# mozilla/mozjpeg

Hardware: AMD Instinct MI355X
Metric: Mpixels/s encode (4K RGB q75 trellis) at 1/2/4/8 GPUs; bit-exact vs cjpeg (higher is better)
Workload: dtype u8/int16 (+f32 trellis costs); 1 GPU; 3840x2160 synthetic RGB, q75 4:2:0 baseline, trellis+deringing+optimal Huffman (cjpeg -quality 75 -baseline); config_key=metric, frames_per_encode_call=96, distinct_frames=96, batches_in_flight=2, input=resident in HBM, output=complete JPEG files in HBM, parallelism=images sharded, 1 process per GPU, no collective

## Files before the change

include/mozjpeg_hip.h:

```cpp
#ifndef MOZJPEG_HIP_H
#define MOZJPEG_HIP_H

#include <stddef.h>
#include <stdint.h>

#ifdef __cplusplus
extern "C" {
#endif

#define MJH_MAX_COMPS 4
#define MJH_MAX_SCANS 64

#define MJH_OK            0
#define MJH_EINVAL       -1
#define MJH_EUNSUPPORTED -2
#define MJH_EHIP         -3
#define MJH_ENOMEM       -4
#define MJH_ETOOSMALL    -5

#define MJH_PROFILE_MAX_COMPRESSION 0x5D083AAD
#define MJH_PROFILE_FASTEST         0x2AEA5CB4

typedef struct {
  int comps_in_scan;
// ... 166 lines not shown
  int dct_method;
  int bottom_up;
  int raw_planes;
  int no_dither;
} mjh_decode_opts;
void mjh_decode_opts_defaults(mjh_decode_opts *o);
int mjh_decode_host(mjh_encoder *e, const void *const jpegs[], const size_t sizes[], int n, const mjh_decode_opts *opts);
int mjh_decode_wait(mjh_encoder *e);
int mjh_get_pixels(mjh_encoder *e, int i, void *dst, size_t row_pitch);
int mjh_get_pixels_device(mjh_encoder *e, void **d_base, size_t *row_pitch, size_t *image_stride);
int mjh_get_plane(mjh_encoder *e, int i, int comp, void *dst, size_t row_pitch, int width, int height);
int mjh_get_planes_device(mjh_encoder *e, int comp, void **d_base, size_t *row_pitch, size_t *image_stride, int *width, int *height);
int mjh_decode_stats(mjh_encoder *e, int *width, int *height, int *pixel_size, float ms[2]);

int mjh_enc_onepass_stats(mjh_encoder *e, int *enabled, unsigned long long *long_blocks, unsigned long long *big_groups);

int mjh_get_jpeg_size(mjh_encoder *e, int i, size_t *size);
int mjh_get_jpeg(mjh_encoder *e, int i, void *dst, size_t cap, size_t *size);
int mjh_get_output_device(mjh_encoder *e, void **d_base, size_t *stride, void **d_sizes);

int mjh_get_scan_table(mjh_encoder *e, int image, int scan, int tblno, uint8_t bits[17], uint8_t vals[256]);

enum {
  MJH_TAP_PLANE = 1,
  MJH_TAP_COEF_UQ = 2,
  MJH_TAP_COEF_Q = 3,
  MJH_TAP_COEF_Q0 = 4,
  MJH_TAP_HUFF_BITS = 5,
  MJH_TAP_HUFF_VALS = 6,
  MJH_TAP_PROG_SCAN_US = 7,
// ... 24 lines not shown
```

mozjpeg_amd/__init__.py:

```python
import ctypes as C
import os

import numpy as np

_HERE = os.path.dirname(os.path.abspath(__file__))
LIB_PATH = os.environ.get("MOZJPEG_AMD_LIB") or os.path.join(_HERE, "libmozjpeg_hip.so")

MAX_COMPS, MAX_SCANS = 4, 64
PROFILE_MAX_COMPRESSION = 0x5D083AAD
PROFILE_FASTEST = 0x2AEA5CB4
COLOR_YCC, COLOR_NONE, COLOR_YCC_IN = 0, 1, 2
CS_GRAYSCALE, CS_RGB, CS_YCBCR = 1, 2, 3
CS_RGB565 = 16
OK, EINVAL, EUNSUPPORTED, EHIP, ENOMEM, ETOOSMALL = 0, -1, -2, -3, -4, -5
TAP_PLANE, TAP_COEF_UQ, TAP_COEF_Q, TAP_COEF_Q0, TAP_HUFF_BITS, TAP_HUFF_VALS, TAP_PROG_SCAN_US, TAP_LL_COUNTS = 1, 2, 3, 4, 5, 6, 7, 8


class MjhError(RuntimeError):
    def __init__(self, code, msg):
        super().__init__("mozjpeg_hip error %d: %s" % (code, msg))
        self.code = code


class Scan(C.Structure):
# ... 127 lines not shown
        L.mjh_transcode_host.argtypes = [C.c_void_p, C.POINTER(C.c_char_p), C.POINTER(C.c_size_t), C.c_int]
        L.mjh_transcode_status.argtypes = [C.c_void_p, C.c_int, C.POINTER(C.c_char_p)]
        L.mjh_transcode_stats.argtypes = [C.c_void_p, C.POINTER(C.c_int), C.POINTER(C.c_int), C.POINTER(C.c_int), C.POINTER(C.c_float)]
        if hasattr(L, "mjh_decode_host"):
            L.mjh_decode_opts_defaults.argtypes = [C.POINTER(DecodeOpts)]
            L.mjh_decode_opts_defaults.restype = None
            L.mjh_decode_host.argtypes = [C.c_void_p, C.POINTER(C.c_char_p), C.POINTER(C.c_size_t), C.c_int, C.POINTER(DecodeOpts)]
            L.mjh_get_pixels.argtypes = [C.c_void_p, C.c_int, C.c_void_p, C.c_size_t]
            L.mjh_get_pixels_device.argtypes = [C.c_void_p, C.POINTER(C.c_void_p), C.POINTER(C.c_size_t), C.POINTER(C.c_size_t)]
            L.mjh_decode_stats.argtypes = [C.c_void_p, C.POINTER(C.c_int), C.POINTER(C.c_int), C.POINTER(C.c_int), C.POINTER(C.c_float)]
            L.mjh_decode_wait.argtypes = [C.c_void_p]
            L.mjh_get_plane.argtypes = [C.c_void_p, C.c_int, C.c_int, C.c_void_p, C.c_size_t, C.c_int, C.c_int]
            L.mjh_get_planes_device.argtypes = [C.c_void_p, C.c_int, C.POINTER(C.c_void_p), C.POINTER(C.c_size_t), C.POINTER(C.c_size_t),
                                                C.POINTER(C.c_int), C.POINTER(C.c_int)]
            L.mjh_transcode_batch_size.argtypes = [C.c_void_p]
        if hasattr(L, "mjh_enc_onepass_stats"):
            L.mjh_enc_onepass_stats.argtypes = [C.c_void_p, C.POINTER(C.c_int), C.POINTER(C.c_ulonglong), C.POINTER(C.c_ulonglong)]
        _lib = L
    return _lib


def _chk(rc):
    if rc != 0:
        raise MjhError(rc, lib().mjh_last_error().decode())


def make_params(width, height, *, quality=75, baseline=False, revert=False, optimize=False,
                notrellis=False, notrellis_dc=False, noovershoot=False, sample=(2, 2), gray=False,
                grayin=False, quant_table=-1, lambda1=None, lambda2=None, restart=None,
                progressive=False, fastcrush=False, precision=8, trellis_loops=1, smooth=0, rgb=False,
# ... 550 lines not shown
    def transcode_status(self, i):
        t = C.c_char_p()
        rc = lib().mjh_transcode_status(self._h, i, C.byref(t))
        return rc, (t.value or b"").decode()

    def transcode_stats(self):
        a, b, c, ms = C.c_int(), C.c_int(), C.c_int(), (C.c_float * 4)()
        _chk(lib().mjh_transcode_stats(self._h, C.byref(a), C.byref(b), C.byref(c), ms))
        return dict(subseq=a.value, rounds=b.value, host_syncs=c.value, ms=dict(zip(("sync", "prefix", "store", "dc"), [float(x) for x in ms])))

    def enc_onepass_stats(self):
        on, a, b = C.c_int(), C.c_ulonglong(), C.c_ulonglong()
        _chk(lib().mjh_enc_onepass_stats(self._h, C.byref(on), C.byref(a), C.byref(b)))
        return dict(enabled=bool(on.value), long_blocks=a.value, big_groups=b.value)

    def transcode_host(self, files, errors="raise", **transform):
        n = len(files)
        if transform:
            self.set_transform(transform_spec(**transform))
        try:
            self.submit_transcode(files)
            return [self.get_jpeg(i) for i in range(n)]
        except MjhError:
            if errors != "return":
                raise
            res = self._file_errors(n)
            if res is None:
                raise
            return res

# ... 127 lines not shown
```

mozjpeg_amd/csrc/mjh_encoder.cpp:

```cpp
#include <hip/hip_runtime.h>

#include <math.h>
#include <stdarg.h>
#include <stdio.h>
#include <stdlib.h>
#include <string.h>

#include <atomic>
#include <condition_variable>
#include <functional>
#include <mutex>
#include <string>
#include <thread>
#include <memory>
#include <chrono>
#include <vector>

#include "../../include/mozjpeg_hip.h"
#include "mjh_internal.h"
#include "mjh_launch.h"
#include "mjh_lossless.h"
#include "mjh_decode.h"
#include "mjh_idct.h"
#include "mjh_guard.h"
// ... 243 lines not shown
  uint8_t *d_planes = nullptr;
  int16_t *d_uq = nullptr, *d_q = nullptr, *d_q0 = nullptr;
  MjhQuant *d_quant = nullptr, *d_quant_init = nullptr;
  MjhHuffTable *d_tabs = nullptr, *d_tabs_init = nullptr;
  float *d_lambda = nullptr;
  uint8_t *d_back = nullptr;
  void *d_eob_cost = nullptr; int *d_eob_has = nullptr; long long *d_qsums = nullptr;
  unsigned long long *d_nzmask = nullptr; bool use_compact = false, compact_last = false;
  size_t small_batch = 400000;
  uint8_t *d_nq8 = nullptr;
  int copy_prio = 0;
  int fastdiv_all = 0;
  int dc_mode = 0;
  int dc_late = 1;
  int dc_stats_side = 1;
  int dc_window_ok = 0;
  int trellis_chunks = 0;
  hipEvent_t ev_chunk[4] = { nullptr, nullptr, nullptr, nullptr };
  int trellis_v3 = 4;
  int dqt_off[4] = { -1, -1, -1, -1 };
  int dqt_tabs[4] = { 0, 0, 0, 0 }, dqt_ntab = 0;
  bool tbl_le1 = true;
  int nbands = 1, freq_split = 8;
  unsigned *d_seg_x = nullptr, *d_seg_E = nullptr, *d_seg_sums = nullptr, *d_seg_totals = nullptr, *d_mpos = nullptr;
  int nseg = 1;
  int comp_restart[4] = { 0, 0, 0, 0 };
  int16_t *d_dense = nullptr; unsigned dense_cap = 0;
  unsigned *d_worklist = nullptr, *d_worklist2 = nullptr;
  int trellis_variant = 0;
  bool trellis_adapt = true;
// ... 542 lines not shown
  if (hipStreamSynchronize(a) != hipSuccess || hipStreamSynchronize(b) != hipSuccess) return -1;
  int votes = 0;
  for (int rep = 0; rep < 3; rep++) {
    const auto t0 = std::chrono::steady_clock::now();
    mjh_launch_spin(15000ull, a);
    mjh_launch_spin(15000ull, b);
    if (hipStreamSynchronize(a) != hipSuccess || hipStreamSynchronize(b) != hipSuccess) return -1;
    const double us = std::chrono::duration<double, std::micro>(std::chrono::steady_clock::now() - t0).count();
    votes += us < 240.0;
  }
  return votes >= 2;
}

static thread_local bool g_create_twin = false;
static thread_local int g_twin_onepass = 1;
static thread_local hipStream_t g_twin_avoid[2] = { nullptr, nullptr };

static hipError_t make_streams(mjh_encoder *e)
{
#define STREAMCHK(x) do { const hipError_t r_ = (x); if (r_ != hipSuccess) return r_; } while (0)
  if (e->high_priority_streams) {
    std::vector<hipStream_t> made;
    for (int tries = 0; tries < 12 && !e->side_stream; tries++) {
      hipStream_t c = nullptr;
      STREAMCHK(hipStreamCreateWithFlags(&c, hipStreamNonBlocking));
      made.push_back(c);
      bool free_queue = true;
      for (hipStream_t other : { g_twin_avoid[0], g_twin_avoid[1], e->stream })
        if (other && mjh_streams_overlap(c, other) == 0) { free_queue = false; break; }
      if (!free_queue) continue;
// ... 129 lines not shown
    HIPCHK_E(mjh_dmalloc((void **)&e->d_dense, (size_t)e->dense_cap * 128));
  }
  {
    double m = 0.0;
    for (int k = 1; k < 64; k++) m += p->quantval[p->quant_tbl_no[0]][k];
    m /= 63.0;
    e->trellis_variant = m >= 38.0 ? 0 : m >= 22.0 ? 2 : m >= 13.0 ? 3 : 4;
  }
  if (const char *v = getenv("MJH_TRELLIS_VARIANT")) { e->trellis_variant = atoi(v); e->trellis_adapt = false; }
  HIPCHK_E(hipHostMalloc((void **)&e->h_defer, 64, hipHostMallocDefault));
  if (const char *v = getenv("MJH_TRELLIS_V3")) e->trellis_v3 = atoi(v);
  if (const char *v = getenv("MJH_SMALL_BATCH")) e->small_batch = (size_t)atoll(v);
  if (const char *v = getenv("MJH_TRELLIS_CHUNKS")) { e->trellis_chunks = atoi(v); if (e->trellis_chunks < 0 || e->trellis_chunks > 4) e->trellis_chunks = 0; }
  for (int i = 0; i < 4; i++) HIPCHK_E(hipEventCreateWithFlags(&e->ev_chunk[i], hipEventDisableTiming));
  if (const char *v = getenv("MJH_DC_LATE")) { e->dc_late = atoi(v); if (e->dc_late < 0 || e->dc_late > 2) e->dc_late = 1; }
  e->dc_window_ok = 1;
  for (int i = 0; i < C.ncomp; i++) if (p->quantval[p->quant_tbl_no[i]][0] < 5) e->dc_window_ok = 0;
  if (const char *v = getenv("MJH_DC_SPEC")) e->dc_spec = atoi(v);
  if (const char *v = getenv("MJH_DECODE_SUBSEQ")) { e->dec_subseq = atoi(v); if (e->dec_subseq < 0 || (e->dec_subseq > 0 && e->dec_subseq < 16)) e->dec_subseq = 16; }
  HIPCHK_E(mjh_dmalloc((void **)&e->d_len16, B * (size_t)C.total_mcu_blocks * 2));
  HIPCHK_E(mjh_dmalloc((void **)&e->d_off32, B * (size_t)C.total_mcu_blocks * 4));
  e->chunks = (C.total_mcu_blocks + 2047) / 2048;
  if (g_create_twin) e->enc_onepass = g_twin_onepass;
  else if (const char *v = getenv("MJH_ENC_ONEPASS")) e->enc_onepass = atoi(v) != 0;
  if (e->enc_onepass) {
    e->pack_words = mjh_encode_pack_words(C);
    HIPCHK_E(mjh_dmalloc((void **)&e->d_pack, B * e->pack_words * 4));
    HIPCHK_E(mjh_dmalloc((void **)&e->d_enc_slow, 2 * sizeof(unsigned)));
    HIPCHK_E(hipMemset(e->d_enc_slow, 0, 2 * sizeof(unsigned)));
  }
// ... 436 lines not shown
}

static int run_lossless(mjh_encoder *e, const void *d_pixels, size_t row_pitch, size_t image_stride, int n, hipStream_t s,
                        hipEvent_t input_read, hipEvent_t before_output);

static int run_pipeline(mjh_encoder *e, const void *d_pixels, size_t row_pitch, size_t image_stride, int n, hipStream_t s,
                        const MjhPlaneSrc *plane_src = nullptr, const MjhCoefSrc *coef_src = nullptr,
                        hipEvent_t input_read = nullptr, hipEvent_t before_output = nullptr)
{
  if (e->lossless) return run_lossless(e, d_pixels, row_pitch, image_stride, n, s, input_read, before_output);
  const MjhConst &C = e->C;
  const mjh_params &p = e->p;
  const int spi = e->spi;
  e->sizes_valid = false;
  e->last_n = n;
  e->res_buf = -1;
  e->coef_input = coef_src != nullptr;
  e->last_stream = s;
  if (!e->owner) e->last = nullptr;
  mjh_encoder *const peer = e->owner ? e->owner : e->twin;
  const int if_mode = peer ? (e->owner ? e->owner : e)->inflight_mode : 0;
  const bool ordered = if_mode >= 1;
  if (if_mode == 1 && peer->ev_tier1_set) HIPCHK(hipStreamWaitEvent(s, peer->ev_tier1, 0));
  e->ev_tier1_set = false;
  const bool peer_done_set = peer && peer->ev_done_set;
  if (if_mode == 2) e->ev_done_set = false;
  Prof pr{ e, s };
  if (e->profiling && e->prof_calls < 256) {
    pr.enabled = true;
    pr.first_call = e->prof_calls == 0;
// ... 142 lines not shown
      mjh_launch_prog_stats_par(C, e->d_prog_scans, e->d_lists + plt->par_off, plt->npar, e->d_prog_ctl, e->d_q, e->d_tabs, spi,
                                e->pe, plt->any_refine, nullptr, n, s, plt->nacf);
      pr.mark("gen_tables(trellis)");
      mjh_launch_gen_tables_list(e->d_tabs, spi, e->d_lists + plt->slot_off, plt->nslot, n, s);
      sl_dc = sl_dc_prog;
    }
    if (e->debug_taps && first_pass) {
      if (!e->d_q0) HIPCHK(mjh_dmalloc((void **)&e->d_q0, (size_t)e->max_batch * C.coefs_per_image * 2));
      HIPCHK(hipMemcpyAsync(e->d_q0, e->d_q, (size_t)n * C.coefs_per_image * 2, hipMemcpyDeviceToDevice, s));
    }
    e->side_timed = false;
    bool dc_late = false;
    const int dc_mode = e->dc_mode;
    if (p.trellis_quant_dc && dc_mode == 1) {
      pr.mark("trellis_dc(serial)");
      mjh_launch_trellis_dc(dc_chain_view(e, CV), e->d_quant, e->d_uq, e->d_q, e->d_tabs, spi, sl_dc, e->d_lambda, e->d_back, n, s, e->dc_window_ok);
    } else if (p.trellis_quant_dc) {
      HIPCHK(hipEventRecord(e->ev_fork, s));
      HIPCHK(hipStreamWaitEvent(e->side_stream, e->ev_fork, 0));
      if (pr.enabled && e->profiling == 1) {
        while (e->side_events.size() < 2 * (size_t)(e->prof_calls + 1)) { hipEvent_t ev; HIPCHK(hipEventCreate(&ev)); e->side_events.push_back(ev); }
        HIPCHK(hipEventRecord(e->side_events[2 * e->prof_calls], e->side_stream));
      }
      const size_t spec_bytes = 2 * (size_t)C.total_real_blocks * 9 * 16;
      const bool spec = e->dc_spec && n <= 2 && qstride == 0 && spec_bytes <= ((size_t)256 << 20) && mjh_trellis_dc_speculative_ok(CV, e->dc_window_ok);
      if (spec && !e->d_back9) {
        int rows = 0;
        for (int c = 0; c < C.ncomp; c++) rows += C.c[c].hib;
        HIPCHK(mjh_dmalloc((void **)&e->d_back9, spec_bytes));
        HIPCHK(mjh_dmalloc((void **)&e->d_jfin, 2 * (size_t)rows * 9 * sizeof(int)));
        HIPCHK(mjh_dmalloc((void **)&e->d_qspec, 2 * (size_t)C.total_real_blocks * 9 * sizeof(int16_t)));
      }
      const bool final_dc_here = !e->progressive && p.optimize_coding && last_loop && nbands == 1 && qstride == 0 && !ext_eob && e->dc_stats_side && e->seq_scans.empty();
      const bool sorted_tier = nzm && e->d_nq8 && e->trellis_v3 > 0 && e->trellis_variant <= 4;
      dc_late = e->dc_late > 0 && sorted_tier && !spec && final_dc_here && nloops == 1 && CV.ncomp == 3 && !e->debug_taps && (size_t)n * C.total_real_blocks >= e->small_batch;
      if (spec) mjh_launch_trellis_dc_speculative(CV, e->d_quant, e->d_uq, e->d_q, e->d_tabs, spi, sl_dc, e->d_lambda, e->d_back9, e->d_jfin, e->d_qspec, n, e->side_stream);
      else
      mjh_launch_trellis_dc(dc_chain_view(e, CV), e->d_quant, e->d_uq, e->d_q, e->d_tabs, spi, sl_dc, e->d_lambda, e->d_back, n, e->side_stream, e->dc_window_ok,
                            0, dc_late ? e->dc_late * CV.mcu_rows : -1);
      if (pr.enabled && e->profiling == 1) { HIPCHK(hipEventRecord(e->side_events[2 * e->prof_calls + 1], e->side_stream)); e->side_timed = true; }
      if (final_dc_here && !dc_late) {
        mjh_launch_stats_dc(C, e->d_q, e->d_tabs, spi, fin_dc, 1, zero4, n, e->side_stream);
        final_dc_counted = true;
      }
      if (!dc_late) HIPCHK(hipEventRecord(e->ev_join, e->side_stream));
    }
    const bool extended = nbands > 1 || ext_eob || qstride != 0;
    if (!extended) { const int rc = adapt_first_tier(); if (rc != MJH_OK) return rc; }
    const bool v3 = nzm && e->d_nq8 && e->trellis_v3 > 0 && e->trellis_variant <= 4 && !extended;
    const bool excl = ordered && v3 && !e->progressive;
    if (excl && peer_done_set) HIPCHK(hipStreamWaitEvent(s, peer->ev_done, 0));
    const int trellis_ranges = !v3 || e->debug_taps || (size_t)n * C.total_real_blocks < e->small_batch ? 1
                               : e->trellis_chunks > 0 ? e->trellis_chunks
                               : !e->progressive && (size_t)n * C.total_real_blocks >= (size_t)6000000 ? 2 : 1;
    const int count_mask = v3 && (size_t)n * C.total_real_blocks >= (size_t)2000000 ? 7 : 0;
    pr.mark("trellis_ac");
    mjh_launch_trellis_ac(CV, e->d_quant, e->d_uq, e->d_q, e->d_tabs, spi, sl_ac, e->d_lambda, e->d_worklist, e->d_worklist2, e->d_dense, e->dense_cap,
                          e->trellis_variant,
                          Ss, Se, ext_eob ? e->d_eob_cost : nullptr, ext_eob ? e->d_eob_has : nullptr, nzm, qstride, n, s,
                          e->d_nq8, v3 ? ((size_t)n * C.total_real_blocks < e->small_batch ? 1 : e->trellis_v3) : 0,
                          e->fastdiv_all, dc_late ? e->ev_side0 : nullptr, excl ? e->ev_tier1 : nullptr,
                          trellis_ranges, e->side_stream, e->ev_chunk, count_mask);
    if (excl) e->ev_tier1_set = true;
    if (dc_late) {
      if (!v3) return fail(MJH_EINVAL, "internal: the late DC chains need the tile-sorted trellis' event");
      HIPCHK(hipStreamWaitEvent(e->side_stream, e->ev_side0, 0));
      mjh_launch_trellis_dc(CV, e->d_quant, e->d_uq, e->d_q, e->d_tabs, spi, sl_dc, e->d_lambda, e->d_back, n, e->side_stream, e->dc_window_ok, e->dc_late * CV.mcu_rows, -1);
      mjh_launch_stats_dc(C, e->d_q, e->d_tabs, spi, fin_dc, 1, zero4, n, e->side_stream);
      final_dc_counted = true;
      HIPCHK(hipEventRecord(e->ev_join, e->side_stream));
      join_late = true;
    }
    if (e->trellis_adapt && !extended && first_pass && !e->defer_pending) {
      if (!e->ev_defer) HIPCHK(hipEventCreateWithFlags(&e->ev_defer, hipEventDisableTiming));
      e->defer_frames = n;
      e->defer_scale = count_mask + 1;
      HIPCHK(hipMemcpyAsync(&e->h_defer[0], e->d_worklist, 4 * sizeof(unsigned), hipMemcpyDeviceToHost, s));
      HIPCHK(hipEventRecord(e->ev_defer, s));
      e->defer_pending = true;
    }
    if (ext_eob) {
      pr.mark("trellis_eob_runs");
// ... 165 lines not shown

static mjh_encoder *cur(mjh_encoder *e) { return e && e->last ? e->last : e; }

extern "C" int mjh_set_inflight(mjh_encoder *e, int batches)
{
  if (!e || batches < 1 || batches > 2) return fail(MJH_EINVAL, "batches in flight: 1 or 2");
  e->inflight = batches;
  return MJH_OK;
}

static int make_twin(mjh_encoder *e)
{
  mjh_encoder *t = nullptr;
  g_create_twin = true;
  g_twin_onepass = e->enc_onepass;
  g_twin_avoid[0] = e->stream; g_twin_avoid[1] = e->side_stream;
  const int rc = mjh_encoder_create(&e->p_created, e->max_batch, e->device, &t);
  g_create_twin = false;
  if (rc) return rc;
  t->owner = e;
  t->inflight = 1;
  t->profiling = e->profiling; t->prof_focus_name = e->prof_focus_name; t->prof_focus = e->prof_focus;
  e->twin = t;
  return MJH_OK;
}

static int wait_pending_pack(mjh_encoder *e, hipStream_t s)
{
  if (e->res_buf >= 0 && !e->res_waited[e->res_buf]) HIPCHK(hipStreamWaitEvent(s, e->ev_packed[e->res_buf], 0));
  return MJH_OK;
// ... 1194 lines not shown
extern "C" int mjh_decode_stats(mjh_encoder *e, int *width, int *height, int *pixel_size, float ms[2])
{
  if (!e) return fail(MJH_EINVAL, "null encoder");
  if (!e->dp_queued) return fail(MJH_EINVAL, "the last batch was not decoded through mjh_decode_host");
  if (width) *width = e->dp.W;
  if (height) *height = e->dp.H;
  if (pixel_size) *pixel_size = e->dp.px_size;
  if (ms) {
    ms[0] = ms[1] = 0.f;
    if (e->dp_timed) {
      HIPCHK(hipSetDevice(e->device));
      HIPCHK(hipEventSynchronize(e->dp_ev[2]));
      for (int k = 0; k < 2; k++) HIPCHK(hipEventElapsedTime(&ms[k], e->dp_ev[k], e->dp_ev[k + 1]));
    }
  }
  return MJH_OK;
}

extern "C" int mjh_enc_onepass_stats(mjh_encoder *e, int *enabled, unsigned long long *long_blocks, unsigned long long *big_groups)
{
  if (!e) return fail(MJH_EINVAL, "null encoder");
  if (enabled) *enabled = e->enc_onepass;
  unsigned long long a = 0, b = 0;
  for (mjh_encoder *x : { e, e->twin }) {
    if (!x || !x->d_enc_slow) continue;
    unsigned h[2] = { 0, 0 };
    HIPCHK(hipSetDevice(x->device));
    HIPCHK(hipDeviceSynchronize());
    HIPCHK(hipMemcpy(h, x->d_enc_slow, sizeof(h), hipMemcpyDeviceToHost));
    a += h[0]; b += h[1];
// ... 492 lines not shown
```

mozjpeg_amd/csrc/mjh_kernels.hip:

```cpp
#include <hip/hip_runtime.h>
#include <stdio.h>
#include <stdlib.h>
#include <stdint.h>
#include <type_traits>
#include <stdlib.h>
#include "mjh_internal.h"
#include "mjh_device.h"

#define WAVE 64

struct ZZTab { int v[64]; };
static constexpr ZZTab make_zz() {
  ZZTab t{};
  const int z[64] = {
    0,  1,  8, 16,  9,  2,  3, 10, 17, 24, 32, 25, 18, 11,  4,  5,
    12, 19, 26, 33, 40, 48, 41, 34, 27, 20, 13,  6,  7, 14, 21, 28,
    35, 42, 49, 56, 57, 50, 43, 36, 29, 22, 15, 23, 30, 37, 44, 51,
    58, 59, 52, 45, 38, 31, 39, 46, 53, 60, 61, 54, 47, 55, 62, 63 };
  for (int i = 0; i < 64; i++) t.v[i] = z[i];
  return t;
}
static constexpr ZZTab kZZ = make_zz();

#define FIXC(x) ((int)((x) * 65536.0 + 0.5))
// ... 1344 lines not shown
#undef DC3_BACK
      if (b >= 0) {
        int cnd = qv - h + myj;
        cnd = min(1023, max(-1023, cnd));
        if (bx < 0) cnd = -cnd;
        qo0[row0 + b] = (int16_t)cnd;
        if (b == cc.wib - 1) last_dc = cnd;
      }
      bx = bx_n; w = w_n;
    }
    last_dc = row_bcast<0>(last_dc);
    __threadfence_block();
  }
}

#define DC3_HYP 9
__global__ void __launch_bounds__(64)
k_trellis_dc3_fwd(MjhConst C, const MjhQuant *__restrict__ Q, const int16_t *__restrict__ coef_uq,
                  const MjhHuffTable *__restrict__ tabs, int slots_per_image, int4 dc_slot_of_comp,
                  const float *__restrict__ lambda_in, uint8_t *__restrict__ back9, int *__restrict__ jfin, int16_t *__restrict__ qspec, int rows_total)
{
  MJH_WAVE_GROUPS(16);
  const int img = blockIdx.y;
  const int lane = threadIdx.x;
  const int k = lane & 15;
  const int chain = blockIdx.x * 4 + (lane >> 4);
  if (chain >= rows_total * DC3_HYP) return;
  const int grow = chain / DC3_HYP, hyp = chain - grow * DC3_HYP;
  int comp = 0, br = grow;
  while (comp + 1 < C.ncomp && br >= C.c[comp].hib) { br -= C.c[comp].hib; comp++; }
// ... 963 lines not shown
bool mjh_trellis_dc_speculative_ok(const MjhConst &C, int window_ok)
{
  return window_ok && C.delta_dc_weight <= 0.0f && C.maxv >= 2;
}

void mjh_launch_trellis_dc_speculative(const MjhConst &C, const MjhQuant *Q, const void *uq, void *q, const MjhHuffTable *tabs, int spi, const int dc_slot[4], const float *lambda,
                                       void *back9, int *jfin, void *qspec, int n, hipStream_t s)
{
  int rows = 0;
  for (int c = 0; c < C.ncomp; c++) rows += C.c[c].hib;
  hipLaunchKernelGGL(k_trellis_dc3_fwd, dim3((rows * DC3_HYP + 3) / 4, n), dim3(64), 0, s, C, Q, (const int16_t *)uq, tabs, spi,
                     make_int4(dc_slot[0], dc_slot[1], dc_slot[2], dc_slot[3]), lambda, (uint8_t *)back9, jfin, (int16_t *)qspec, rows);
  hipLaunchKernelGGL(k_trellis_dc3_resolve, dim3(C.ncomp * C.mcu_rows, n), dim3(64), 0, s, C, (int16_t *)q, (const int *)jfin, (const int16_t *)qspec, rows);
}

void mjh_launch_trellis_dc(const MjhConst &C, const MjhQuant *Q, const void *uq, void *q, const MjhHuffTable *tabs, int spi, const int dc_slot[4], const float *lambda, void *back, int n, hipStream_t s,
                           int window_ok, int chain0, int chain1)
{
  const int nchains = C.ncomp * C.mcu_rows;
  if (chain1 < 0 || chain1 > nchains) chain1 = nchains;
  if (chain0 >= chain1) return;
  dim3 grid((chain1 - chain0 + 3) / 4, n);
  if (window_ok && C.delta_dc_weight <= 0.0f)
    hipLaunchKernelGGL(k_trellis_dc3, grid, dim3(64), 0, s, C, Q, (const int16_t *)uq, (int16_t *)q, tabs, spi, make_int4(dc_slot[0], dc_slot[1], dc_slot[2], dc_slot[3]), lambda, (uint8_t *)back, chain0, chain1);
  else hipLaunchKernelGGL(k_trellis_dc2, grid, dim3(64), 0, s, C, Q, (const int16_t *)uq, (int16_t *)q, tabs, spi, make_int4(dc_slot[0], dc_slot[1], dc_slot[2], dc_slot[3]), lambda, (uint8_t *)back, chain0, chain1);
}

void mjh_launch_encode(const MjhConst &C, const void *q, const unsigned long long *nzmask, const MjhHuffTable *tabs, int spi, const int dc_slot[4], const int ac_slot[4],
                       void *len16, void *off32, unsigned *sums, int chunks_per_image, unsigned *totals,
                       unsigned *stream, size_t stream_words_per_image, void *meta,
                       unsigned *seg_x, unsigned *seg_E, unsigned *seg_sums, unsigned *seg_totals, unsigned *mpos, int nseg,
                       int n, hipStream_t s, unsigned *pack, size_t pack_words_per_image, unsigned *slow)
{
  const int4 ds = make_int4(dc_slot[0], dc_slot[1], dc_slot[2], dc_slot[3]);
  const int4 as = make_int4(ac_slot[0], ac_slot[1], ac_slot[2], ac_slot[3]);
  if (pack && C.restart_interval == 0) {
    const int segs = mjh_encode_segments(C);
    dim3 gridp(segs, n);
    if (nzmask) hipLaunchKernelGGL((k_enc_write_pack<true>), gridp, dim3(256), 0, s, C, (const int16_t *)q, nzmask, tabs, spi, ds, as, pack, pack_words_per_image, sums, segs,
                                   (MjhImageMeta *)meta, slow);
// ... 76 lines not shown
```

mozjpeg_amd/csrc/mjh_launch.h:

```cpp
#ifndef MJH_LAUNCH_H
#define MJH_LAUNCH_H
#include <hip/hip_runtime.h>
#include "mjh_internal.h"

void mjh_launch_import_coefs(const MjhConst &C, const MjhCoefSrc &S, void *coef_q, void *meta, int n, hipStream_t s);
void mjh_launch_import_planes(const MjhConst &C, const MjhPlaneSrc &S, void *planes, int n, hipStream_t s);
void mjh_launch_color(const MjhConst &C, const void *pix, size_t row_pitch, size_t img_stride, void *planes, int n, hipStream_t s);
void mjh_launch_dct(const MjhConst &C, const MjhQuant *Q, const void *planes, void *uq, void *q, float *lambda,
                    MjhHuffTable *stat_tabs, int spi, const int stat_slot[4], uint8_t *nq8, int n, hipStream_t s, int fastdiv = 0, int ifast = 0);
void mjh_launch_stats_ac(const MjhConst &C, const void *q, const unsigned long long *nzmask, MjhHuffTable *tabs, int spi, const int slot[4], int count_dummies, int n, hipStream_t s);
void mjh_launch_stats_dc(const MjhConst &C, const void *q, MjhHuffTable *tabs, int spi, const int slot[4], int mcu_order, const int comp_restart[4], int n, hipStream_t s);
void mjh_launch_gen_tables(MjhHuffTable *tabs, int spi, const int *slots, int nslots, int n, hipStream_t s);
void mjh_launch_trellis_ac(const MjhConst &C, const MjhQuant *Q, const void *uq, void *q, MjhHuffTable *tabs, int spi, const int ac_slot[4], const float *lambda,
                           unsigned *worklist, unsigned *worklist2, void *dense, unsigned dense_cap, int variant,
                           int Ss, int Se, void *eob_cost, int *eob_has, unsigned long long *nzmask, int qstride, int n, hipStream_t s,
                           uint8_t *nq8 = nullptr, int v3_passes = 0, int fastdiv = 0, hipEvent_t after_first_tier = nullptr, hipEvent_t after_first_tier2 = nullptr,
                           int chunks = 1, hipStream_t side = nullptr, hipEvent_t *ev_chunk = nullptr, int count_mask = 0);
void mjh_launch_trellis_eob_chain(const MjhConst &C, void *q, const MjhHuffTable *tabs, int spi, const int ac_slot[4], const void *eob_cost, const int *eob_has,
                                  int Ss, int Se, int n, hipStream_t s);
void mjh_launch_qopt_accumulate(const MjhConst &C, const void *uq, const void *q, void *sums, int n, hipStream_t s);
void mjh_launch_qopt_update(void *sums, MjhQuant *Q, int n, hipStream_t s);
void mjh_launch_qopt_fix(const MjhQuant *Q, void *out, size_t out_stride, unsigned *sizes, int dqt_start, int sof_off, const int *tabs, int ntab,
                         int multi, int baseline_capable, int n, hipStream_t s);
void mjh_launch_trellis_dc(const MjhConst &C, const MjhQuant *Q, const void *uq, void *q, const MjhHuffTable *tabs, int spi, const int dc_slot[4], const float *lambda, void *back, int n, hipStream_t s,
                           int window_ok = 0, int chain0 = 0, int chain1 = -1);
void mjh_launch_encode(const MjhConst &C, const void *q, const unsigned long long *nzmask, const MjhHuffTable *tabs, int spi, const int dc_slot[4], const int ac_slot[4],
                       void *len16, void *off32, unsigned *sums, int chunks_per_image, unsigned *totals,
                       unsigned *stream, size_t stream_words_per_image, void *meta,
                       unsigned *seg_x, unsigned *seg_E, unsigned *seg_sums, unsigned *seg_totals, unsigned *mpos, int nseg,
                       int n, hipStream_t s, unsigned *pack = nullptr, size_t pack_words_per_image = 0, unsigned *slow = nullptr);
int mjh_encode_segments(const MjhConst &C);
size_t mjh_encode_pack_words(const MjhConst &C);
void mjh_launch_header(const void *prefix, int prefix_len, const void *sos, int sos_len, const MjhHuffTable *tabs, int spi,
                       const int dht_slots[8], const int dht_ids[8], int ndht, int multi_dht, void *out, size_t out_stride, void *meta, int n, hipStream_t s, const unsigned *append_sizes = nullptr);
void mjh_launch_finish_bits(unsigned *totals, unsigned *stream, size_t stream_words_per_image, void *meta, int n, hipStream_t s);
void mjh_launch_stuff(const unsigned *stream, size_t stream_words_per_image, const unsigned *totals, unsigned *ffsums, int ff_chunks_per_image,
                      unsigned *ff_totals, void *out, size_t out_stride, void *meta, unsigned *sizes, const unsigned *mpos, int nseg, int n, hipStream_t s);
void mjh_launch_pack_results(const void *out, size_t out_stride, const unsigned *sizes, const void *meta, const void *prog_ctl, int n,
                             void *dst, size_t cap, void *table, hipStream_t s);
void mjh_launch_spin(unsigned long long ticks_100mhz, hipStream_t s);
// ... 27 lines not shown
```

Before: 148,700 Mpixels/s.

## Add one-thread-per-chain DC trellis kernel for large batches

Adds a new DC trellis kernel, k_trellis_dc_lane, in which each thread runs the Viterbi forward pass and the backtrack for one MCU-row chain. It uses templated candidate counts, vectorised loads of coefficients and lambda, and packed back-pointer stores. The launcher picks it over the wave-per-4-chains dc3/dc2 kernels when the window condition holds and batch*mcu_rows reaches a threshold (12000 by default, settable with MJH_DC_LANES). The aim is to fill the GPU with many independent serial chains at large batch sizes instead of spending whole waves on few chains. The trade-off is long serial per-thread loops and uncoalesced per-thread memory access. A query API reporting which DC path ran is also added.

```diff
diff --git a/include/mozjpeg_hip.h b/include/mozjpeg_hip.h
--- a/include/mozjpeg_hip.h
+++ b/include/mozjpeg_hip.h
@@ -204,6 +204,7 @@
 int mjh_decode_stats(mjh_encoder *e, int *width, int *height, int *pixel_size, float ms[2]);
 
 int mjh_enc_onepass_stats(mjh_encoder *e, int *enabled, unsigned long long *long_blocks, unsigned long long *big_groups);
+int mjh_get_dc_path(mjh_encoder *e, int *path);
 
 int mjh_get_jpeg_size(mjh_encoder *e, int i, size_t *size);
 int mjh_get_jpeg(mjh_encoder *e, int i, void *dst, size_t cap, size_t *size);
diff --git a/mozjpeg_amd/__init__.py b/mozjpeg_amd/__init__.py
--- a/mozjpeg_amd/__init__.py
+++ b/mozjpeg_amd/__init__.py
@@ -165,6 +165,8 @@
             L.mjh_get_planes_device.argtypes = [C.c_void_p, C.c_int, C.POINTER(C.c_void_p), C.POINTER(C.c_size_t), C.POINTER(C.c_size_t),
                                                 C.POINTER(C.c_int), C.POINTER(C.c_int)]
             L.mjh_transcode_batch_size.argtypes = [C.c_void_p]
+        if hasattr(L, "mjh_get_dc_path"):
+            L.mjh_get_dc_path.argtypes = [C.c_void_p, C.POINTER(C.c_int)]
         if hasattr(L, "mjh_enc_onepass_stats"):
             L.mjh_enc_onepass_stats.argtypes = [C.c_void_p, C.POINTER(C.c_int), C.POINTER(C.c_ulonglong), C.POINTER(C.c_ulonglong)]
         _lib = L
@@ -745,6 +747,11 @@
         _chk(lib().mjh_enc_onepass_stats(self._h, C.byref(on), C.byref(a), C.byref(b)))
         return dict(enabled=bool(on.value), long_blocks=a.value, big_groups=b.value)
 
+    def dc_path(self):
+        v = C.c_int()
+        _chk(lib().mjh_get_dc_path(self._h, C.byref(v)))
+        return (None, "lane", "dc3", "dc2", "speculative")[v.value]
+
     def transcode_host(self, files, errors="raise", **transform):
         n = len(files)
         if transform:
diff --git a/mozjpeg_amd/csrc/mjh_encoder.cpp b/mozjpeg_amd/csrc/mjh_encoder.cpp
--- a/mozjpeg_amd/csrc/mjh_encoder.cpp
+++ b/mozjpeg_amd/csrc/mjh_encoder.cpp
@@ -281,6 +281,9 @@
   int dc_mode = 0;
   int dc_late = 1;
   int dc_stats_side = 1;
+  int dc_lanes = 12000;
+  int dc_lanes_set = 0;
+  int dc_path = 0;
   int dc_window_ok = 0;
   int trellis_chunks = 0;
   hipEvent_t ev_chunk[4] = { nullptr, nullptr, nullptr, nullptr };
@@ -853,6 +856,7 @@
 
 static thread_local bool g_create_twin = false;
 static thread_local int g_twin_onepass = 1;
+static thread_local int g_twin_dc_lanes = 0, g_twin_dc_lanes_set = 0;
 static thread_local hipStream_t g_twin_avoid[2] = { nullptr, nullptr };
 
 static hipError_t make_streams(mjh_encoder *e)
@@ -1012,6 +1016,8 @@
   if (const char *v = getenv("MJH_TRELLIS_CHUNKS")) { e->trellis_chunks = atoi(v); if (e->trellis_chunks < 0 || e->trellis_chunks > 4) e->trellis_chunks = 0; }
   for (int i = 0; i < 4; i++) HIPCHK_E(hipEventCreateWithFlags(&e->ev_chunk[i], hipEventDisableTiming));
   if (const char *v = getenv("MJH_DC_LATE")) { e->dc_late = atoi(v); if (e->dc_late < 0 || e->dc_late > 2) e->dc_late = 1; }
+  if (g_create_twin) { e->dc_lanes = g_twin_dc_lanes; e->dc_lanes_set = g_twin_dc_lanes_set; }
+  else if (const char *v = getenv("MJH_DC_LANES")) { e->dc_lanes = atoi(v); if (e->dc_lanes < 0) e->dc_lanes = 0; e->dc_lanes_set = 1; }
   e->dc_window_ok = 1;
   for (int i = 0; i < C.ncomp; i++) if (p->quantval[p->quant_tbl_no[i]][0] < 5) e->dc_window_ok = 0;
   if (const char *v = getenv("MJH_DC_SPEC")) e->dc_spec = atoi(v);
@@ -1478,6 +1484,7 @@
   const int spi = e->spi;
   e->sizes_valid = false;
   e->last_n = n;
+  e->dc_path = MJH_DC_PATH_NONE;
   e->res_buf = -1;
   e->coef_input = coef_src != nullptr;
   e->last_stream = s;
@@ -1650,7 +1657,7 @@
     const int dc_mode = e->dc_mode;
     if (p.trellis_quant_dc && dc_mode == 1) {
       pr.mark("trellis_dc(serial)");
-      mjh_launch_trellis_dc(dc_chain_view(e, CV), e->d_quant, e->d_uq, e->d_q, e->d_tabs, spi, sl_dc, e->d_lambda, e->d_back, n, s, e->dc_window_ok);
+      e->dc_path = mjh_launch_trellis_dc(dc_chain_view(e, CV), e->d_quant, e->d_uq, e->d_q, e->d_tabs, spi, sl_dc, e->d_lambda, e->d_back, n, s, e->dc_window_ok, 0, -1, e->dc_lanes);
     } else if (p.trellis_quant_dc) {
       HIPCHK(hipEventRecord(e->ev_fork, s));
       HIPCHK(hipStreamWaitEvent(e->side_stream, e->ev_fork, 0));
@@ -1659,7 +1666,8 @@
         HIPCHK(hipEventRecord(e->side_events[2 * e->prof_calls], e->side_stream));
       }
       const size_t spec_bytes = 2 * (size_t)C.total_real_blocks * 9 * 16;
-      const bool spec = e->dc_spec && n <= 2 && qstride == 0 && spec_bytes <= ((size_t)256 << 20) && mjh_trellis_dc_speculative_ok(CV, e->dc_window_ok);
+      const bool spec = e->dc_spec && n <= 2 && qstride == 0 && spec_bytes <= ((size_t)256 << 20) && mjh_trellis_dc_speculative_ok(CV, e->dc_window_ok) &&
+                        !(e->dc_lanes_set && mjh_trellis_dc_lanes_ok(dc_chain_view(e, CV), e->dc_window_ok, n, e->dc_lanes));
       if (spec && !e->d_back9) {
         int rows = 0;
         for (int c = 0; c < C.ncomp; c++) rows += C.c[c].hib;
@@ -1670,10 +1678,10 @@
       const bool final_dc_here = !e->progressive && p.optimize_coding && last_loop && nbands == 1 && qstride == 0 && !ext_eob && e->dc_stats_side && e->seq_scans.empty();
       const bool sorted_tier = nzm && e->d_nq8 && e->trellis_v3 > 0 && e->trellis_variant <= 4;
       dc_late = e->dc_late > 0 && sorted_tier && !spec && final_dc_here && nloops == 1 && CV.ncomp == 3 && !e->debug_taps && (size_t)n * C.total_real_blocks >= e->small_batch;
-      if (spec) mjh_launch_trellis_dc_speculative(CV, e->d_quant, e->d_uq, e->d_q, e->d_tabs, spi, sl_dc, e->d_lambda, e->d_back9, e->d_jfin, e->d_qspec, n, e->side_stream);
+      if (spec) { mjh_launch_trellis_dc_speculative(CV, e->d_quant, e->d_uq, e->d_q, e->d_tabs, spi, sl_dc, e->d_lambda, e->d_back9, e->d_jfin, e->d_qspec, n, e->side_stream); e->dc_path = MJH_DC_PATH_SPEC; }
       else
-      mjh_launch_trellis_dc(dc_chain_view(e, CV), e->d_quant, e->d_uq, e->d_q, e->d_tabs, spi, sl_dc, e->d_lambda, e->d_back, n, e->side_stream, e->dc_window_ok,
-                            0, dc_late ? e->dc_late * CV.mcu_rows : -1);
+      e->dc_path = mjh_launch_trellis_dc(dc_chain_view(e, CV), e->d_quant, e->d_uq, e->d_q, e->d_tabs, spi, sl_dc, e->d_lambda, e->d_back, n, e->side_stream, e->dc_window_ok,
+                            0, dc_late ? e->dc_late * CV.mcu_rows : -1, e->dc_lanes);
       if (pr.enabled && e->profiling == 1) { HIPCHK(hipEventRecord(e->side_events[2 * e->prof_calls + 1], e->side_stream)); e->side_timed = true; }
       if (final_dc_here && !dc_late) {
         mjh_launch_stats_dc(C, e->d_q, e->d_tabs, spi, fin_dc, 1, zero4, n, e->side_stream);
@@ -1701,7 +1709,7 @@
     if (dc_late) {
       if (!v3) return fail(MJH_EINVAL, "internal: the late DC chains need the tile-sorted trellis' event");
       HIPCHK(hipStreamWaitEvent(e->side_stream, e->ev_side0, 0));
-      mjh_launch_trellis_dc(CV, e->d_quant, e->d_uq, e->d_q, e->d_tabs, spi, sl_dc, e->d_lambda, e->d_back, n, e->side_stream, e->dc_window_ok, e->dc_late * CV.mcu_rows, -1);
+      mjh_launch_trellis_dc(CV, e->d_quant, e->d_uq, e->d_q, e->d_tabs, spi, sl_dc, e->d_lambda, e->d_back, n, e->side_stream, e->dc_window_ok, e->dc_late * CV.mcu_rows, -1, e->dc_lanes);
       mjh_launch_stats_dc(C, e->d_q, e->d_tabs, spi, fin_dc, 1, zero4, n, e->side_stream);
       final_dc_counted = true;
       HIPCHK(hipEventRecord(e->ev_join, e->side_stream));
@@ -1897,6 +1905,7 @@
   mjh_encoder *t = nullptr;
   g_create_twin = true;
   g_twin_onepass = e->enc_onepass;
+  g_twin_dc_lanes = e->dc_lanes; g_twin_dc_lanes_set = e->dc_lanes_set;
   g_twin_avoid[0] = e->stream; g_twin_avoid[1] = e->side_stream;
   const int rc = mjh_encoder_create(&e->p_created, e->max_batch, e->device, &t);
   g_create_twin = false;
@@ -3121,6 +3130,14 @@
       for (int k = 0; k < 2; k++) HIPCHK(hipEventElapsedTime(&ms[k], e->dp_ev[k], e->dp_ev[k + 1]));
     }
   }
+  return MJH_OK;
+}
+
+extern "C" int mjh_get_dc_path(mjh_encoder *e, int *path)
+{
+  if (!e || !path) return fail(MJH_EINVAL, "null argument");
+  const mjh_encoder *x = e->last ? e->last : e;
+  *path = x->dc_path;
   return MJH_OK;
 }
 
diff --git a/mozjpeg_amd/csrc/mjh_kernels.hip b/mozjpeg_amd/csrc/mjh_kernels.hip
--- a/mozjpeg_amd/csrc/mjh_kernels.hip
+++ b/mozjpeg_amd/csrc/mjh_kernels.hip
@@ -1382,6 +1382,177 @@
   }
 }
 
+#ifndef DCL_BLOCK
+#define DCL_BLOCK 128
+#endif
+#ifndef DCL_G
+#define DCL_G 8
+#endif
+template <int NC> __device__ __forceinline__ float dc_lane_min(const float (&c)[NC])
+{
+  float m = fminf(fminf(c[0], c[1]), c[2]);
+  if constexpr (NC == 5) m = fminf(fminf(m, c[3]), c[4]);
+  if constexpr (NC >= 7) {
+    const float m1 = fminf(fminf(c[3], c[4]), c[5]);
+    if constexpr (NC == 7) m = fminf(fminf(m, m1), c[6]);
+    else m = fminf(fminf(m, m1), fminf(fminf(c[6], c[7]), c[8]));
+  }
+  return m;
+}
+template <int NC>
+__device__ __forceinline__ void dc_lane_chain(const MjhComp &cc, int imcu, unsigned long long rsi, int dq, float rcp, float lt0,
+                                              const int16_t *__restrict__ uq0, int16_t *__restrict__ qo0, const float *__restrict__ lam, uint4 *__restrict__ bk)
+{
+  constexpr int N1 = NC - 1, H = NC / 2;
+  int last_dc = 0;
+  for (int sub = 0; sub < cc.v; sub++) {
+    const int br = imcu * cc.v + sub;
+    if (br >= cc.hib) break;
+    const int row0 = br * cc.wib;
+    float pc[NC];
+    pc[0] = 0.0f;
+#pragma unroll
+    for (int i = 1; i < NC; i++) pc[i] = 3e38f;
+    int prev_c0 = last_dc, R = 0;
+    struct alignas(2) XsG { int16_t v[DCL_G]; };
+    struct alignas(4) LamG { float v[DCL_G]; };
+    struct alignas(8) BackG { uint2 v[DCL_G]; };
+    uint2 *bk8 = reinterpret_cast<uint2 *>(bk);
+    auto fetch = [&](int g, XsG &xo, LamG &lo) {
+      if (g + DCL_G <= cc.wib) {
+        __builtin_memcpy(&xo, uq0 + row0 + g, sizeof(XsG));
+        __builtin_memcpy(&lo, lam + row0 + g, sizeof(LamG));
+      } else {
+#pragma unroll
+        for (int s = 0; s < DCL_G; s++) { const int b = min(g + s, cc.wib - 1); xo.v[s] = uq0[row0 + b]; lo.v[s] = lam[row0 + b]; }
+      }
+    };
+    XsG xs_c, xs_n;
+    LamG lam_c, lam_n;
+    fetch(0, xs_c, lam_c);
+    for (int g = 0; g < cc.wib; g += DCL_G) {
+      fetch(g + DCL_G, xs_n, lam_n);
+      BackG bw;
+#pragma unroll
+      for (int s = 0; s < DCL_G; s++) {
+        bw.v[s] = make_uint2(0, 0);
+        if (g + s < cc.wib) {
+          const int xs = xs_c.v[s];
+          const float lambda_dc = lam_c.v[s] * lt0;
+          const int x = xs < 0 ? -xs : xs, neg = xs < 0 ? 1 : 0;
+          const int qv = udiv_exact(x + (dq >> 1), dq, rcp);
+          const int c0 = neg ? -(qv + H) : qv - H;
+          const int D = c0 - prev_c0, Dp = R ? -D : D;
+          const int flip = neg ^ R;
+          float rt[2 * NC - 1];
+#pragma unroll
+          for (int t = 0; t < 2 * NC - 1; t++) rt[t] = dc_rate(rsi, Dp + t - N1);
+          const int dA = mul24(qv - H + (flip ? N1 : 0), dq) - x, stq = flip ? -dq : dq;
+          float best[NC];
+          unsigned lo = 0, hi = 0;
+#pragma unroll
+          for (int a = 0; a < NC; a++) {
+            const int delta = dA + mul24(a, stq);
+            const float dist = (float)mul24(delta, delta) * lambda_dc;
+            float c[NC];
+#pragma unroll
+            for (int i = 0; i < NC; i++) c[i] = pc[i] + (rt[a - i + N1] + dist);
+            const float m = dc_lane_min<NC>(c);
+            int bb = N1;
+#pragma unroll
+            for (int i = N1 - 1; i >= 0; i--) bb = c[i] == m ? i : bb;
+            best[a] = m;
+            if (a < 8) lo |= (unsigned)bb << (4 * a); else hi = (unsigned)bb;
+          }
+#pragma unroll
+          for (int k = 0; k < NC; k++) pc[k] = flip ? best[N1 - k] : best[k];
+          prev_c0 = c0;
+          R = neg;
+          hi |= (unsigned)flip << 4 | (unsigned)neg << 5 | (unsigned)((qv - H) & 0xFFFF) << 16;
+          bw.v[s] = make_uint2(lo, hi);
+        }
+      }
+      if (g + DCL_G <= cc.wib && ((row0 + g) & 1) == 0) {
+#pragma unroll
+        for (int s = 0; s < DCL_G; s += 2) *reinterpret_cast<uint4 *>(bk8 + row0 + g + s) = make_uint4(bw.v[s].x, bw.v[s].y, bw.v[s + 1].x, bw.v[s + 1].y);
+      } else
+#pragma unroll
+        for (int s = 0; s < DCL_G; s++) if (g + s < cc.wib) bk8[row0 + g + s] = bw.v[s];
+      xs_c = xs_n; lam_c = lam_n;
+    }
+    int j = N1;
+    {
+      const float m = dc_lane_min<NC>(pc);
+#pragma unroll
+      for (int i = N1 - 1; i >= 0; i--) j = pc[i] == m ? i : j;
+    }
+    __threadfence_block();
+    auto fetch_back = [&](int top, BackG &wo) {
+      if (top - (DCL_G - 1) >= 0 && ((row0 + top - (DCL_G - 1)) & 1) == 0) {
+#pragma unroll
+        for (int s = 0; s < DCL_G; s += 2) {
+          const uint4 q = *reinterpret_cast<const uint4 *>(bk8 + row0 + top - (DCL_G - 1) + s);
+          wo.v[s] = make_uint2(q.x, q.y); wo.v[s + 1] = make_uint2(q.z, q.w);
+        }
+      } else
+#pragma unroll
+        for (int s = 0; s < DCL_G; s++) wo.v[s] = bk8[row0 + max(top - (DCL_G - 1) + s, 0)];
+    };
+    BackG w_c, w_n;
+    fetch_back(cc.wib - 1, w_c);
+    for (int top = cc.wib - 1; top >= 0; top -= DCL_G) {
+      fetch_back(top - DCL_G, w_n);
+      XsG out;
+#pragma unroll
+      for (int s = DCL_G - 1; s >= 0; s--) {
+        out.v[s] = 0;
+        if (top - (DCL_G - 1) + s >= 0) {
+          const uint2 w = w_c.v[s];
+          int cnd = (int)(short)(w.y >> 16) + j;
+          if (w.y & 32u) cnd = -cnd;
+          out.v[s] = (int16_t)cnd;
+          if (s == DCL_G - 1 && top == cc.wib - 1) last_dc = cnd;
+          const int a = (w.y & 16u) ? N1 - j : j;
+          j = (int)(((((unsigned long long)w.y) << 32 | w.x) >> (4 * a)) & 15u);
+        }
+      }
+      if (top - (DCL_G - 1) >= 0) __builtin_memcpy(qo0 + row0 + top - (DCL_G - 1), &out, sizeof(XsG));
+      else
+#pragma unroll
+        for (int s = 0; s < DCL_G; s++) if (top - (DCL_G - 1) + s >= 0) qo0[row0 + top - (DCL_G - 1) + s] = out.v[s];
+      w_c = w_n;
+    }
+  }
+}
+
+__global__ void __launch_bounds__(DCL_BLOCK)
+k_trellis_dc_lane(MjhConst C, const MjhQuant *__restrict__ Q, const int16_t *__restrict__ coef_uq,
+                  int16_t *__restrict__ coef_q, const MjhHuffTable *__restrict__ tabs, int slots_per_image,
+                  int slot, const float *__restrict__ lambda_in, uint8_t *__restrict__ back, int comp, int imcu0, int cnt, int total)
+{
+  const int t = blockIdx.x * DCL_BLOCK + threadIdx.x;
+  if (t >= total) return;
+  const int img = t / cnt, imcu = imcu0 + (t - img * cnt);
+  const MjhComp cc = C.c[comp];
+  const MjhHuffTable *T = tabs + (size_t)img * slots_per_image + slot;
+  unsigned long long rsi = 0;
+  for (int s = 0; s < 12; s++) rsi |= (unsigned long long)((T->ehufsi[s] + s) & 31) << (5 * s);
+  const int q0 = Q->q[cc.qtbl][0];
+  const int dq = 8 * q0;
+  const float rcp = Q->rcp8q[cc.qtbl][0];
+  const float lt0 = Q->lambda_tbl[cc.qtbl][0];
+  int ncand = (2 + 60 / q0) | 1;
+  if (ncand > 9) ncand = 9;
+  const int16_t *uq0 = coef_uq + (size_t)img * C.coefs_per_image + cc.coef_off;
+  int16_t *qo0 = coef_q + (size_t)img * C.coefs_per_image + cc.coef_off;
+  const float *lam = lambda_in + (size_t)img * C.total_real_blocks + cc.blk_off;
+  uint4 *bk = reinterpret_cast<uint4 *>(back) + ((size_t)img * C.total_real_blocks + cc.blk_off);
+  if (ncand == 9) dc_lane_chain<9>(cc, imcu, rsi, dq, rcp, lt0, uq0, qo0, lam, bk);
+  else if (ncand == 7) dc_lane_chain<7>(cc, imcu, rsi, dq, rcp, lt0, uq0, qo0, lam, bk);
+  else if (ncand == 5) dc_lane_chain<5>(cc, imcu, rsi, dq, rcp, lt0, uq0, qo0, lam, bk);
+  else dc_lane_chain<3>(cc, imcu, rsi, dq, rcp, lt0, uq0, qo0, lam, bk);
+}
+
 #define DC3_HYP 9
 __global__ void __launch_bounds__(64)
 k_trellis_dc3_fwd(MjhConst C, const MjhQuant *__restrict__ Q, const int16_t *__restrict__ coef_uq,
@@ -2375,16 +2546,34 @@
   hipLaunchKernelGGL(k_trellis_dc3_resolve, dim3(C.ncomp * C.mcu_rows, n), dim3(64), 0, s, C, (int16_t *)q, (const int *)jfin, (const int16_t *)qspec, rows);
 }
 
-void mjh_launch_trellis_dc(const MjhConst &C, const MjhQuant *Q, const void *uq, void *q, const MjhHuffTable *tabs, int spi, const int dc_slot[4], const float *lambda, void *back, int n, hipStream_t s,
-                           int window_ok, int chain0, int chain1)
+bool mjh_trellis_dc_lanes_ok(const MjhConst &C, int window_ok, int n, int lanes_min)
+{
+  return window_ok && C.delta_dc_weight <= 0.0f && lanes_min > 0 && (long long)n * C.mcu_rows >= lanes_min;
+}
+
+int mjh_launch_trellis_dc(const MjhConst &C, const MjhQuant *Q, const void *uq, void *q, const MjhHuffTable *tabs, int spi, const int dc_slot[4], const float *lambda, void *back, int n, hipStream_t s,
+                          int window_ok, int chain0, int chain1, int lanes_min)
 {
   const int nchains = C.ncomp * C.mcu_rows;
   if (chain1 < 0 || chain1 > nchains) chain1 = nchains;
-  if (chain0 >= chain1) return;
+  if (chain0 >= chain1) return MJH_DC_PATH_NONE;
+  if (mjh_trellis_dc_lanes_ok(C, window_ok, n, lanes_min)) {
+    for (int c = 0; c < C.ncomp; c++) {
+      const int lo = chain0 > c * C.mcu_rows ? chain0 : c * C.mcu_rows, hi = chain1 < (c + 1) * C.mcu_rows ? chain1 : (c + 1) * C.mcu_rows;
+      if (lo >= hi) continue;
+      const int cnt = hi - lo, total = n * cnt;
+      hipLaunchKernelGGL(k_trellis_dc_lane, dim3((total + DCL_BLOCK - 1) / DCL_BLOCK), dim3(DCL_BLOCK), 0, s, C, Q, (const int16_t *)uq, (int16_t *)q, tabs, spi, dc_slot[c], lambda, (uint8_t *)back,
+                         c, lo - c * C.mcu_rows, cnt, total);
+    }
+    return MJH_DC_PATH_LANE;
+  }
   dim3 grid((chain1 - chain0 + 3) / 4, n);
-  if (window_ok && C.delta_dc_weight <= 0.0f)
+  if (window_ok && C.delta_dc_weight <= 0.0f) {
     hipLaunchKernelGGL(k_trellis_dc3, grid, dim3(64), 0, s, C, Q, (const int16_t *)uq, (int16_t *)q, tabs, spi, make_int4(dc_slot[0], dc_slot[1], dc_slot[2], dc_slot[3]), lambda, (uint8_t *)back, chain0, chain1);
-  else hipLaunchKernelGGL(k_trellis_dc2, grid, dim3(64), 0, s, C, Q, (const int16_t *)uq, (int16_t *)q, tabs, spi, make_int4(dc_slot[0], dc_slot[1], dc_slot[2], dc_slot[3]), lambda, (uint8_t *)back, chain0, chain1);
+    return MJH_DC_PATH_DC3;
+  }
+  hipLaunchKernelGGL(k_trellis_dc2, grid, dim3(64), 0, s, C, Q, (const int16_t *)uq, (int16_t *)q, tabs, spi, make_int4(dc_slot[0], dc_slot[1], dc_slot[2], dc_slot[3]), lambda, (uint8_t *)back, chain0, chain1);
+  return MJH_DC_PATH_DC2;
 }
 
 void mjh_launch_encode(const MjhConst &C, const void *q, const unsigned long long *nzmask, const MjhHuffTable *tabs, int spi, const int dc_slot[4], const int ac_slot[4],
diff --git a/mozjpeg_amd/csrc/mjh_launch.h b/mozjpeg_amd/csrc/mjh_launch.h
--- a/mozjpeg_amd/csrc/mjh_launch.h
+++ b/mozjpeg_amd/csrc/mjh_launch.h
@@ -22,8 +22,10 @@
 void mjh_launch_qopt_update(void *sums, MjhQuant *Q, int n, hipStream_t s);
 void mjh_launch_qopt_fix(const MjhQuant *Q, void *out, size_t out_stride, unsigned *sizes, int dqt_start, int sof_off, const int *tabs, int ntab,
                          int multi, int baseline_capable, int n, hipStream_t s);
-void mjh_launch_trellis_dc(const MjhConst &C, const MjhQuant *Q, const void *uq, void *q, const MjhHuffTable *tabs, int spi, const int dc_slot[4], const float *lambda, void *back, int n, hipStream_t s,
-                           int window_ok = 0, int chain0 = 0, int chain1 = -1);
+enum { MJH_DC_PATH_NONE = 0, MJH_DC_PATH_LANE = 1, MJH_DC_PATH_DC3 = 2, MJH_DC_PATH_DC2 = 3, MJH_DC_PATH_SPEC = 4 };
+bool mjh_trellis_dc_lanes_ok(const MjhConst &C, int window_ok, int n, int lanes_min);
+int mjh_launch_trellis_dc(const MjhConst &C, const MjhQuant *Q, const void *uq, void *q, const MjhHuffTable *tabs, int spi, const int dc_slot[4], const float *lambda, void *back, int n, hipStream_t s,
+                          int window_ok = 0, int chain0 = 0, int chain1 = -1, int lanes_min = 0);
 void mjh_launch_encode(const MjhConst &C, const void *q, const unsigned long long *nzmask, const MjhHuffTable *tabs, int spi, const int dc_slot[4], const int ac_slot[4],
                        void *len16, void *off32, unsigned *sums, int chunks_per_image, unsigned *totals,
                        unsigned *stream, size_t stream_words_per_image, void *meta,
```

After: 155,500 Mpixels/s (median of 6 runs). 1.05x the previous value.
